# ak110/object_detector

Hardware: AMD Instinct MI355X
Metric: images_per_sec (higher is better)
Workload: dtype f16

## Files before the change

object_detector_amd/csrc/conv_8ph_kernel.h:

```cpp
#pragma once
#include "conv_8ph_tile.h"
#include "conv_common.h"

namespace {

constexpr int E_ALO = 0, E_AHI = E_REGION, E_BLO = 2 * E_REGION, E_BHI = 3 * E_REGION;

struct TapWalk {
  int c0, tap, tapoff, dx;
  int sel_tap;
};

constexpr unsigned E_OOB = 0x80000000u;

template <int MT, int NF = 4, bool KEEP = false>
static __device__ __forceinline__ void e8_epilogue_rt(const ConvKP& p, f32x4 (&acc)[MT][NF], int m0w, int n0w, int l15,
                                                          int lq, f16x8 (*keep)[NF / 2] = nullptr, int mrows = MT * 16,
                                                          const float* pre_sc = nullptr, const float* pre_bi = nullptr) {
  unsigned pb[MT], ppix[MT];
#pragma unroll
  for (int i = 0; i < MT; ++i) {
    const int m = m0w + i * 16 + l15;
    pb[i] = (unsigned)m / (unsigned)p.HoWo;
    ppix[i] = (unsigned)m - pb[i] * (unsigned)p.HoWo;
  }
#pragma unroll
  for (int pr = 0; pr < NF / 2; ++pr) {
    const int n = n0w + (2 * pr + (lq & 1)) * 16 + (lq >> 1) * 8;
    const bool nok = n < p.Cout;
    float sc[8], bi[8];
    if (pre_sc) {
#pragma unroll
      for (int e = 0; e < 8; ++e) {
        sc[e] = pre_sc[e];
        bi[e] = pre_bi[e];
      }
    } else {
      const f32x4 s0 = *(const f32x4*)(p.scale + n), s1 = *(const f32x4*)(p.scale + n + 4);
      const f32x4 b0 = *(const f32x4*)(p.bias + n), b1 = *(const f32x4*)(p.bias + n + 4);
#pragma unroll
      for (int e = 0; e < 4; ++e) {
        sc[e] = s0[e];
        sc[4 + e] = s1[e];
        bi[e] = b0[e];
        bi[4 + e] = b1[e];
      }
    }
    f16x8 rv[MT];
#pragma unroll
    for (int i = 0; i < MT; ++i) {
      const int m = m0w + i * 16 + l15;
      f16x8 r = {0, 0, 0, 0, 0, 0, 0, 0};
      if (nok && m < p.M && p.res_mode != OD_RES_NONE) {
        long long roff;
        if (p.res_mode == OD_RES_SAME) {
          roff = (long long)m * p.Cout + n;
        } else {
          const unsigned ho = ppix[i] / (unsigned)p.Wo, wo = ppix[i] - ho * (unsigned)p.Wo;
          roff = ((long long)(pb[i] * (unsigned)(p.Ho >> 1) + (ho >> 1)) * (p.Wo >> 1) + (wo >> 1)) * p.Cout + n;
        }
        r = *(const f16x8*)(p.res + roff);
      }
      rv[i] = r;
    }
#pragma unroll
    for (int i = 0; i < MT; ++i) {
      const int m = m0w + i * 16 + l15;
      const bool ok = nok && m < p.M && i * 16 + l15 < mrows;
      float v[8];
#pragma unroll
      for (int e = 0; e < 4; ++e) {
        float a = acc[i][2 * pr][e], bq = acc[i][2 * pr + 1][e];
        od_permlane16_swap(a, bq);
        v[e] = a;
        v[4 + e] = bq;
      }
#pragma unroll
      for (int e = 0; e < 8; ++e) v[e] = v[e] * sc[e] + bi[e];
      if (p.act == OD_ACT_LEAKY) {
#pragma unroll
        for (int e = 0; e < 8; ++e) v[e] = od_leaky(v[e], p.alpha);
      } else if (p.act == OD_ACT_ELU) {
#pragma unroll
        for (int e = 0; e < 8; ++e) v[e] = v[e] > 0.f ? v[e] : p.alpha * od_expm1_fast(v[e]);
      }
      if (p.res_mode != OD_RES_NONE) {
#pragma unroll
        for (int e = 0; e < 8; ++e) v[e] += (float)rv[i][e];
      }
      if (ok) {
        const long long ooff = (long long)pb[i] * p.obs + (long long)ppix[i] * p.ops + n;
        if (p.out_f32) {
          float* o = (float*)p.out + ooff;
          *(f32x4*)o = f32x4{v[0], v[1], v[2], v[3]};
          *(f32x4*)(o + 4) = f32x4{v[4], v[5], v[6], v[7]};
        } else {
          f16x8 h;
#pragma unroll
          for (int e = 0; e < 8; ++e) h[e] = (f16)v[e];
          *(f16x8*)((f16*)p.out + ooff) = h;
        }
      }
      if (KEEP) {
        f16x8 h;
#pragma unroll
        for (int e = 0; e < 8; ++e) h[e] = (f16)v[e];
        keep[i][pr] = h;
      }
    }
  }
}

template <int EPI, int MT, int NF, bool KEEP>
static __device__ __forceinline__ void e8_epilogue_fixed(const ConvKP& p, f32x4 (&acc)[MT][NF], int m0w, int n0w, int l15, int lq,
                                                         f16x8 (*keep)[NF / 2], int mrows, const float* pre_sc,
                                                         const float* pre_bi) {
  constexpr int ACT = od_epi_act(EPI), RES = od_epi_res(EPI);
  constexpr bool F32 = od_epi_f32(EPI);
  unsigned orow[MT], rrow[RES != OD_RES_NONE ? MT : 1];
#pragma unroll
  for (int i = 0; i < MT; ++i) {
    const unsigned m = (unsigned)min(m0w + i * 16 + l15, p.M - 1);
    const unsigned b = m / (unsigned)p.HoWo, pix = m - b * (unsigned)p.HoWo;
    orow[i] = b * (unsigned)p.obs + pix * (unsigned)p.ops;
    if (RES == OD_RES_SAME) rrow[i] = m * (unsigned)p.Cout;
    if (RES == OD_RES_UP2) {
      const unsigned ho = pix / (unsigned)p.Wo, wo = pix - ho * (unsigned)p.Wo;
      rrow[i] = ((b * (unsigned)(p.Ho >> 1) + (ho >> 1)) * (unsigned)(p.Wo >> 1) + (wo >> 1)) * (unsigned)p.Cout;
    }
  }
#pragma unroll
  for (int pr = 0; pr < NF / 2; ++pr) {
    const int n = n0w + (2 * pr + (lq & 1)) * 16 + (lq >> 1) * 8;
    const bool nok = n < p.Cout;
    float sc[8], bi[8];
    if (pre_sc) {
#pragma unroll
      for (int e = 0; e < 8; ++e) {
        sc[e] = pre_sc[e];
        bi[e] = pre_bi[e];
      }
    } else {
      const f32x4 s0 = *(const f32x4*)(p.scale + n), s1 = *(const f32x4*)(p.scale + n + 4);
      const f32x4 b0 = *(const f32x4*)(p.bias + n), b1 = *(const f32x4*)(p.bias + n + 4);
#pragma unroll
      for (int e = 0; e < 4; ++e) {
        sc[e] = s0[e];
        sc[4 + e] = s1[e];
        bi[e] = b0[e];
        bi[4 + e] = b1[e];
      }
    }
    f16x8 rv[RES != OD_RES_NONE ? MT : 1];
    if (RES != OD_RES_NONE) {
      const unsigned nr = nok ? (unsigned)n : 0u;
#pragma unroll
      for (int i = 0; i < MT; ++i) rv[i] = *(const f16x8*)(p.res + (rrow[i] + nr));
    }
#pragma unroll
    for (int i = 0; i < MT; ++i) {
      f32x4 a = acc[i][2 * pr], bq = acc[i][2 * pr + 1];
      od_permlane16_swap4(a, bq);
      float v[8] = {a[0], a[1], a[2], a[3], bq[0], bq[1], bq[2], bq[3]};
#pragma unroll
      for (int e = 0; e < 8; ++e) v[e] = v[e] * sc[e] + bi[e];
      if (ACT == OD_ACT_LEAKY) {
#pragma unroll
        for (int e = 0; e < 8; ++e) v[e] = od_leaky(v[e], p.alpha);
      } else if (ACT == OD_ACT_ELU) {
#pragma unroll
        for (int e = 0; e < 8; ++e) v[e] = od_elu_select(v[e], p.alpha);
      }
      if (RES != OD_RES_NONE) {
#pragma unroll
        for (int e = 0; e < 8; ++e) v[e] += (float)rv[i][e];
      }
      f16x8 h;
      if (!F32 || KEEP) {
#pragma unroll
        for (int e = 0; e < 8; ++e) h[e] = (f16)v[e];
      }
      if (nok && m0w + i * 16 + l15 < p.M && i * 16 + l15 < mrows) {
        const unsigned ooff = orow[i] + (unsigned)n;
        if (F32) {
          float* o = (float*)p.out + ooff;
          *(f32x4*)o = f32x4{v[0], v[1], v[2], v[3]};
          *(f32x4*)(o + 4) = f32x4{v[4], v[5], v[6], v[7]};
        } else {
          *(f16x8*)((f16*)p.out + ooff) = h;
        }
      }
      if (KEEP) keep[i][pr] = h;
    }
  }
}

template <int MT, int NF = 4, bool KEEP = false, int EPI = OD_EPI_RT>
static __device__ __forceinline__ void e8_epilogue_direct(const ConvKP& p, f32x4 (&acc)[MT][NF], int m0w, int n0w, int l15,
                                                          int lq, f16x8 (*keep)[NF / 2] = nullptr, int mrows = MT * 16,
                                                          const float* pre_sc = nullptr, const float* pre_bi = nullptr) {
  if constexpr (EPI == OD_EPI_RT)
    e8_epilogue_rt<MT, NF, KEEP>(p, acc, m0w, n0w, l15, lq, keep, mrows, pre_sc, pre_bi);
  else
    e8_epilogue_fixed<EPI, MT, NF, KEEP>(p, acc, m0w, n0w, l15, lq, keep, mrows, pre_sc, pre_bi);
}

template <int KS, int MF1, int EPI, int EPI2, bool PW, bool SEG>
__global__ __launch_bounds__(512, 2) void od_conv_8ph(ConvKP p_in) {
  constexpr int MF0 = 4, MT = MF0 + MF1, WROWS = MT * 16, BM = 2 * WROWS;
  extern __shared__ __attribute__((aligned(16))) char smem[];
  const int tid = threadIdx.x;
  const int lane = tid & 63;
  const int wave = __builtin_amdgcn_readfirstlane(tid >> 6);
  const int wr = wave >> 2, wc = wave & 3;
  const int l15 = lane & 15, lq = lane >> 4;

  int logical;
  {
    const int nt = p_in.mtiles * p_in.ntiles;
    const int pid = p_in.splitk > 1 ? (int)blockIdx.x / p_in.splitk : (int)blockIdx.x;
    const int q = nt >> 3, r = nt & 7, xcd = pid & 7, loc = pid >> 3;
    logical = (xcd < r ? xcd * (q + 1) : r * (q + 1) + (xcd - r) * q) + loc;
  }
  int tm = logical / p_in.ntiles;
  const int tn = logical - tm * p_in.ntiles;
  ConvKP p_seg;
  if (SEG) p_seg = p_in;
  if (SEG && p_in.nseg > 1) {
    int sg = 0;
    if (tm >= p_in.seg_tile0[1]) sg = 1;
    if (p_in.nseg > 2 && tm >= p_in.seg_tile0[2]) sg = 2;
    tm -= p_in.seg_tile0[sg];
    p_seg.x = p_in.seg_x[sg];
    p_seg.out = p_in.seg_out[sg];
    p_seg.H = p_seg.Ho = p_in.seg_H[sg];
    p_seg.W = p_seg.Wo = p_in.seg_W[sg];
    p_seg.HoWo = p_seg.H * p_seg.W;
    p_seg.M = p_in.seg_M[sg];
    p_seg.x_bytes = (unsigned)p_seg.M * (unsigned)p_in.Cin * 2u;
    if (p_in.obs == 0) p_seg.obs = (long long)p_seg.HoWo * p_in.Cout;
  }
  const ConvKP& p = SEG ? p_seg : p_in;
  const int m0 = tm * BM, n0 = tn * E_BN;
  const int nk_all = p.Ktot / E_BK;
  const int ks0 = p.splitk > 1 ? ((int)blockIdx.x % p.splitk) * p.steps_per_split : 0;
  const int nk = p.splitk > 1 ? min(p.steps_per_split, nk_all - ks0) : nk_all;
  if (nk <= 0) return;

  const int rr = tid >> 3;
  const int lc = (tid & 7) ^ (rr & 7);
  int a_base[2][2];
  unsigned a_vmask[2][2];
  unsigned a_sel[2][2];
#pragma unroll
  for (int s = 0; s < 2; ++s)
#pragma unroll
    for (int j = 0; j < 2; ++j) {
      const int m = m0 + j * WROWS + s * 64 + rr;
      a_vmask[s][j] = 0u;
      a_base[s][j] = 0;
      if (m < p.M && (s == 0 || rr < MF1 * 16)) {
        const unsigned b = (unsigned)m / (unsigned)p.HoWo;
        const unsigned pix = (unsigned)m - b * (unsigned)p.HoWo;
        const unsigned ho = pix / (unsigned)p.Wo;
        const unsigned wo = pix - ho * (unsigned)p.Wo;
        const int hi0 = (int)ho * p.stride - p.pad, wi0 = (int)wo * p.stride - p.pad;
        a_base[s][j] = ((((int)b * p.H + hi0 + p.pad) * p.W + wi0 + p.pad) * p.Cin + lc * 8) * 2;
#pragma unroll
        for (int t = 0; t < KS * KS; ++t) {
          const int hi = hi0 + t / KS, wi = wi0 + t % KS;
          if ((unsigned)hi < (unsigned)p.H && (unsigned)wi < (unsigned)p.W) a_vmask[s][j] |= 1u << t;
        }
      }
    }
  int w_off[2][2];
#pragma unroll
  for (int s = 0; s < 2; ++s)
#pragma unroll
    for (int j = 0; j < 2; ++j) {
      const int n = n0 + (2 * j + (rr >> 5)) * 64 + s * 32 + (rr & 31);
      w_off[s][j] = (n * p.Kstride + lc * 8 + ks0 * E_BK) * 2;
    }
  const __amdgpu_buffer_rsrc_t rs_x = __builtin_amdgcn_make_buffer_rsrc(
      (void*)(p.x - (long long)p.pad * (p.W + 1) * p.Cin), 0, (int)(p.x_bytes + (unsigned)(p.pad * (p.W + 1) * p.Cin * 2)),
      0x00020000);
  const __amdgpu_buffer_rsrc_t rs_w = __builtin_amdgcn_make_buffer_rsrc((void*)p.w, 0, (int)p.w_bytes, 0x00020000);
  auto blds16 = [&](const __amdgpu_buffer_rsrc_t& rs, unsigned voff, int soff, char* lptr) {
    __builtin_amdgcn_raw_ptr_buffer_load_lds(rs, (__attribute__((address_space(3))) void*)lptr, 16, (int)voff, soff, 0, 0);
  };

  auto walk_init = [&](TapWalk& w, int kt) {
    const int k0 = kt * E_BK;
    if (KS == 3) {
      w.sel_tap = -1;
      w.tap = k0 / p.Cin;
      w.c0 = k0 - w.tap * p.Cin;
      const int dy = w.tap / 3;
      w.dx = w.tap - dy * 3;
      w.tapoff = (dy * p.W + w.dx) * p.Cin;
    } else {
      w.sel_tap = -1;
      w.tap = 0;
      w.c0 = k0;
      w.dx = 0;
      w.tapoff = 0;
    }
  };
  auto walk_next = [&](TapWalk& w) {
    w.c0 += E_BK;
    if (KS == 3 && w.c0 >= p.Cin) {
      w.c0 = 0;
      ++w.tap;
      if (++w.dx == 3) {
        w.dx = 0;
        w.tapoff += (p.W - 2) * p.Cin;
      } else {
        w.tapoff += p.Cin;
      }
    }
  };
  TapWalk walk_lo, walk_hi;
  walk_init(walk_lo, ks0);
  walk_init(walk_hi, ks0);

  char* const piece = smem + wave * 1024;
  auto stage_a = [&](int s, TapWalk& w, int buf) {
    const int koff = w.tapoff + w.c0;
    char* dst = piece + buf * E_BUF + (s ? E_AHI : E_ALO);
    if (w.sel_tap != w.tap) {
      w.sel_tap = w.tap;
#pragma unroll
      for (int j = 0; j < 2; ++j) a_sel[s][j] = ((a_vmask[s][j] >> w.tap) & 1u) ? (unsigned)a_base[s][j] : E_OOB;
    }
#pragma unroll
    for (int j = 0; j < 2; ++j) blds16(rs_x, a_sel[s][j], koff * 2, dst + j * 8192);
    walk_next(w);
  };
  auto stage_b = [&](int s, int t, int buf) {
    char* dst = piece + buf * E_BUF + (s ? E_BHI : E_BLO);
#pragma unroll
    for (int j = 0; j < 2; ++j) blds16(rs_w, (unsigned)w_off[s][j], t * (E_BK * 2), dst + j * 8192);
  };

  const int w2buf = ((nk - 1) & 1) ^ 1;
  const __amdgpu_buffer_rsrc_t rs_w2 =
      __builtin_amdgcn_make_buffer_rsrc((void*)(PW ? p.w2 : p.w), 0, (int)(PW ? p.w2_bytes : p.w_bytes), 0x00020000);
  auto stage_w2 = [&](int ks) {
#pragma unroll
    for (int h = 0; h < 2; ++h)
      blds16(rs_w2, (unsigned)(((h * 64 + rr) * p.K2stride + lc * 8) * 2), ks * (E_BK * 2),
             piece + w2buf * E_BUF + ks * E_REGION + h * 8192);
  };

  f32x4 acc[MT][4];
#pragma unroll
  for (int i = 0; i < MT; ++i)
#pragma unroll
    for (int j = 0; j < 4; ++j) acc[i][j] = f32x4{0.f, 0.f, 0.f, 0.f};

  stage_a(0, walk_lo, 0);
  stage_b(0, 0, 0);
  stage_b(1, 0, 0);
  stage_a(1, walk_hi, 0);
  if (nk > 1) {
    stage_a(0, walk_lo, 1);
    stage_b(0, 1, 1);
    wait_vmcnt<8>();
  } else {
    wait_vmcnt<0>();
  }
  __builtin_amdgcn_s_barrier();

  const int fa = (wr * 64 + l15) * 128 + ((lq ^ (l15 & 7)) * 16);
  const int fb = (wc * 32 + l15) * 128 + ((lq ^ (l15 & 7)) * 16);

  f16x8 xa[MF0][2], wlo[2][2], whi[2][2];
  auto ldf = [&](f16x8& dst, const char* src) { dst = *(const f16x8*)src; };
  auto mma = [&](f32x4& c, const f16x8& a, const f16x8& b) {
    c = __builtin_amdgcn_mfma_f32_16x16x32_f16(a, b, c, 0, 0, 0);
  };

  auto L0 = [&](int t) {
    const char* cur = smem + (t & 1) * E_BUF;
#pragma unroll
    for (int f = 0; f < 2; ++f)
#pragma unroll
      for (int kh = 0; kh < 2; ++kh) ldf(wlo[f][kh], cur + E_BLO + ((fb + f * 2048) ^ (kh * 64)));
#pragma unroll
    for (int f = 0; f < MF0; ++f)
#pragma unroll
      for (int kh = 0; kh < 2; ++kh) ldf(xa[f][kh], cur + E_ALO + ((fa + f * 2048) ^ (kh * 64)));
    if (t + 1 < nk) {
      stage_b(1, t + 1, (t & 1) ^ 1);
      wait_vmcnt<8>();
    } else if (PW) {
      stage_w2(0);
      wait_vmcnt<2>();
    } else {
      wait_vmcnt<0>();
    }
  };
  auto L1 = [&](int t) {
    const char* cur = smem + (t & 1) * E_BUF;
#pragma unroll
    for (int f = 0; f < 2; ++f)
#pragma unroll
      for (int kh = 0; kh < 2; ++kh) ldf(whi[f][kh], cur + E_BHI + ((fb + f * 2048) ^ (kh * 64)));
    if (t + 1 < nk) {
      stage_a(1, walk_hi, (t & 1) ^ 1);
      wait_vmcnt<8>();
    } else if (PW) {
      stage_w2(1);
    } else {
      wait_vmcnt<0>();
    }
  };
  auto L2 = [&](int t) {
    const char* cur = smem + (t & 1) * E_BUF;
#pragma unroll
    for (int f = 0; f < MF1; ++f)
#pragma unroll
      for (int kh = 0; kh < 2; ++kh) ldf(xa[f][kh], cur + E_AHI + ((fa + f * 2048) ^ (kh * 64)));
    if (t + 2 < nk) stage_a(0, walk_lo, t & 1);
    if (PW && t + 1 == nk) stage_w2(2);
  };
  auto L3 = [&](int t) {
    if (t + 2 < nk) {
      stage_b(0, t + 2, t & 1);
      wait_vmcnt<8>();
    } else if (PW && t + 1 == nk) {
      stage_w2(3);
    } else {
      wait_vmcnt<0>();
    }
  };
  auto M = [&](int ph) {
    __builtin_amdgcn_s_setprio(1);
#pragma unroll
    for (int kh = 0; kh < 2; ++kh)
#pragma unroll
      for (int i = 0; i < ((ph < 2) ? MF0 : MF1); ++i)
#pragma unroll
        for (int j = 0; j < 2; ++j) {
          if (ph == 0) mma(acc[i][j], wlo[j][kh], xa[i][kh]);
          if (ph == 1) mma(acc[i][2 + j], whi[j][kh], xa[i][kh]);
          if (ph == 2) mma(acc[MF0 + i][2 + j], whi[j][kh], xa[i][kh]);
          if (ph == 3) mma(acc[MF0 + i][j], wlo[j][kh], xa[i][kh]);
        }
    __builtin_amdgcn_s_setprio(0);
  };

  if (wr == 0) {
    for (int t = 0; t < nk; ++t) {
      L0(t);
      M(0);
      __builtin_amdgcn_s_barrier();
      L1(t);
      M(1);
      __builtin_amdgcn_s_barrier();
      L2(t);
      M(2);
      __builtin_amdgcn_s_barrier();
      L3(t);
      M(3);
      __builtin_amdgcn_s_barrier();
    }
  } else {
    L0(0);
    __builtin_amdgcn_s_barrier();
    for (int t = 0; t < nk; ++t) {
      M(0);
      L1(t);
      __builtin_amdgcn_s_barrier();
      M(1);
      L2(t);
      __builtin_amdgcn_s_barrier();
      M(2);
      L3(t);
      __builtin_amdgcn_s_barrier();
      M(3);
      if (t + 1 < nk) {
        L0(t + 1);
        __builtin_amdgcn_s_barrier();
      }
    }
  }
  __syncthreads();

  if constexpr (PW) {
    const int rg = wave >> 2, cg = wave & 3;
    float sc2[8], bi2[8];
    {
      const int n2 = cg * 32 + (lq & 1) * 16 + (lq >> 1) * 8;
      const f32x4 s0 = *(const f32x4*)(p.scale2 + n2), s1 = *(const f32x4*)(p.scale2 + n2 + 4);
      const f32x4 b0 = *(const f32x4*)(p.bias2 + n2), b1 = *(const f32x4*)(p.bias2 + n2 + 4);
#pragma unroll
      for (int e = 0; e < 4; ++e) {
        sc2[e] = s0[e];
        sc2[4 + e] = s1[e];
        bi2[e] = b0[e];
        bi2[4 + e] = b1[e];
      }
    }
    f16x8 ykeep[MT][2];
    od_mfma_results_ready();
    e8_epilogue_direct<MT, 4, true, EPI>(p, acc, m0 + wr * WROWS, n0 + wc * 64, l15, lq, ykeep);
    ConvKP p2 = p;
    p2.scale = p.scale2;
    p2.bias = p.bias2;
    p2.act = p.act2;
    p2.alpha = p.alpha2;
    p2.res_mode = OD_RES_NONE;
    p2.out = (void*)p.out2;
    p2.out_f32 = 0;
    p2.Cout = p.Cout2;
    p2.obs = (long long)p.HoWo * p.Cout2;
    p2.ops = p.Cout2;
    char* const ybuf = smem + (w2buf ^ 1) * E_BUF;
    const char* const wbuf = smem + w2buf * E_BUF;
    const int fy = (rg * 64 + l15) * 128 + ((lq ^ (l15 & 7)) * 16);
    const int fw = (cg * 32 + l15) * 128 + ((lq ^ (l15 & 7)) * 16);
#pragma unroll
    for (int half = 0; half < 2; ++half) {
      if (wr == half) {
#pragma unroll
        for (int i = 0; i < MT; ++i)
#pragma unroll
          for (int pr = 0; pr < 2; ++pr) {
            const int row = i * 16 + l15;
            const int chunk = (2 * pr + (lq & 1)) * 2 + (lq >> 1);
            *(f16x8*)(ybuf + wc * E_REGION + row * 128 + ((chunk ^ (row & 7)) * 16)) = ykeep[i][pr];
          }
      }
      asm volatile("s_waitcnt lgkmcnt(0)" ::: "memory");
      __builtin_amdgcn_s_barrier();
      f32x4 acc2[4][2];
#pragma unroll
      for (int i = 0; i < 4; ++i)
#pragma unroll
        for (int f = 0; f < 2; ++f) acc2[i][f] = f32x4{0.f, 0.f, 0.f, 0.f};
#pragma unroll
      for (int ks = 0; ks < 4; ++ks)
#pragma unroll
        for (int kh = 0; kh < 2; ++kh) {
          f16x8 wf[2], yf[4];
#pragma unroll
          for (int f = 0; f < 2; ++f) wf[f] = *(const f16x8*)(wbuf + ks * E_REGION + ((fw + f * 2048) ^ (kh * 64)));
#pragma unroll
          for (int i = 0; i < 4; ++i) yf[i] = *(const f16x8*)(ybuf + ks * E_REGION + ((fy + i * 2048) ^ (kh * 64)));
#pragma unroll
          for (int i = 0; i < 4; ++i)
#pragma unroll
            for (int f = 0; f < 2; ++f) acc2[i][f] = __builtin_amdgcn_mfma_f32_16x16x32_f16(wf[f], yf[i], acc2[i][f], 0, 0, 0);
        }
      od_mfma_results_ready();
      e8_epilogue_direct<4, 2, false, EPI2>(p2, acc2, m0 + half * WROWS + rg * 64, cg * 32, l15, lq, nullptr, WROWS - rg * 64, sc2, bi2);
      if (half == 0) {
        asm volatile("s_waitcnt lgkmcnt(0)" ::: "memory");
        __builtin_amdgcn_s_barrier();
      }
    }
  } else if (EPI == OD_EPI_RT && p.splitk > 1) {
    conv_epilogue<E_BN, 2, 4, MT, 4, 512>(p, smem, acc, m0, n0, tid, wr, wc, l15, lq);
  } else {
    od_mfma_results_ready();
    e8_epilogue_direct<MT, 4, false, EPI>(p, acc, m0 + wr * WROWS, n0 + wc * 64, l15, lq);
  }
}

}
```

object_detector_amd/csrc/conv_common.h:

```cpp
#pragma once
#include "common.h"

struct ConvKP {
  const f16* x;
  const f16* w;
  const float* scale;
  const float* bias;
  const f16* res;
  void* out;
  const f16* zero;
  int H, W, Cin, Ho, Wo, Cout;
  int stride, pad;
  int Kstride, Ktot, M, HoWo;
  int act;
  float alpha;
  int res_mode, out_f32;
  long long obs, ops;
  int mtiles, ntiles;
  int splitk, steps_per_split;
  float* ws;
  int Mq;
  int tconv, Hs, Ws;
  unsigned x_bytes, w_bytes;
  float* stats;
  const f16* w2;
  const float* scale2;
  const float* bias2;
  f16* out2;
  int Cout2, act2;
  float alpha2;
  unsigned w2_bytes;
  int K2stride;
  int nseg;
  int seg_tile0[4];
  const f16* seg_x[3];
  void* seg_out[3];
  int seg_H[3], seg_W[3], seg_M[3];
  int off32;
};

static __device__ __forceinline__ void glds16(const void* gptr, void* lptr) {
  __builtin_amdgcn_global_load_lds((const __attribute__((address_space(1))) void*)gptr,
                                   (__attribute__((address_space(3))) void*)lptr, 16, 0, 0);
}

static __device__ __forceinline__ float od_expm1_fast(float v) {
  const float poly = v * (1.f + v * (0.5f + v * (1.f / 6 + v * (1.f / 24 + v * (1.f / 120 + v * (1.f / 720))))));
  return v > -0.25f ? poly : __expf(v) - 1.f;
}

static __device__ __forceinline__ float od_elu_select(float v, float alpha) {
  const float poly = v * (1.f + v * (0.5f + v * (1.f / 6 + v * (1.f / 24 + v * (1.f / 120 + v * (1.f / 720))))));
  const float ex = __expf(v) - 1.f;
  const float em = v > -0.25f ? poly : ex;
  const float neg = alpha * em;
  return v > 0.f ? v : neg;
}

#define OD_EPI_RT -1
#define OD_EPI_LEAKY_NONE_F16 1
#define OD_EPI_LEAKY_SAME_F16 5
#define OD_EPI_ELU_NONE_F16 2
#define OD_EPI_ELU_UP2_F16 10
#define OD_EPI_LINEAR_NONE_F32 16
#define OD_EPI_LEAKY_NONE_F32 17
#define OD_EPI_ELU_NONE_F32 18
constexpr int od_epi(int act, int res_mode, bool out_f32) { return act | (res_mode << 2) | ((int)out_f32 << 4); }
static_assert(od_epi(OD_ACT_LEAKY, OD_RES_NONE, false) == OD_EPI_LEAKY_NONE_F16 &&
                  od_epi(OD_ACT_LEAKY, OD_RES_SAME, false) == OD_EPI_LEAKY_SAME_F16 &&
                  od_epi(OD_ACT_ELU, OD_RES_NONE, false) == OD_EPI_ELU_NONE_F16 &&
                  od_epi(OD_ACT_ELU, OD_RES_UP2, false) == OD_EPI_ELU_UP2_F16 &&
                  od_epi(OD_ACT_LINEAR, OD_RES_NONE, true) == OD_EPI_LINEAR_NONE_F32 &&
                  od_epi(OD_ACT_LEAKY, OD_RES_NONE, true) == OD_EPI_LEAKY_NONE_F32 &&
                  od_epi(OD_ACT_ELU, OD_RES_NONE, true) == OD_EPI_ELU_NONE_F32,
              "OD_EPI_* literals");
constexpr int od_epi_act(int epi) { return epi & 3; }
constexpr int od_epi_res(int epi) { return (epi >> 2) & 3; }
constexpr bool od_epi_f32(int epi) { return ((epi >> 4) & 1) != 0; }
static inline int od_epi_of(const ConvKP& p) {
  return (p.off32 && p.splitk <= 1 && !p.tconv && !p.stats) ? od_epi(p.act, p.res_mode, p.out_f32 != 0) : OD_EPI_RT;
}
#define OD_STR_(x) #x
#define OD_STR(x) OD_STR_(x)

static __device__ __forceinline__ void od_permlane16_swap(float& a, float& b) {
  asm volatile("s_nop 1\n\tv_permlane16_swap_b32 %0, %1\n\ts_nop 1" : "+v"(a), "+v"(b));
}
static __device__ __forceinline__ void od_permlane16_swap4(f32x4& a, f32x4& b) {
  float a0 = a[0], a1 = a[1], a2 = a[2], a3 = a[3], b0 = b[0], b1 = b[1], b2 = b[2], b3 = b[3];
  asm volatile(
      "s_nop 1\n\tv_permlane16_swap_b32 %0, %4\n\tv_permlane16_swap_b32 %1, %5\n\tv_permlane16_swap_b32 %2, %6\n\t"
      "v_permlane16_swap_b32 %3, %7\n\ts_nop 1"
      : "+v"(a0), "+v"(a1), "+v"(a2), "+v"(a3), "+v"(b0), "+v"(b1), "+v"(b2), "+v"(b3));
  a = f32x4{a0, a1, a2, a3};
  b = f32x4{b0, b1, b2, b3};
}
static __device__ __forceinline__ void od_mfma_results_ready() {
  __builtin_amdgcn_sched_barrier(0);
  asm volatile("s_nop 15\n\ts_nop 15" ::: "memory");
  __builtin_amdgcn_sched_barrier(0);
}

static __device__ __forceinline__ float od_leaky(float v, float alpha) { return fmaxf(v, v * alpha); }

template <int N>
static __device__ __forceinline__ void wait_vmcnt() {
  asm volatile("s_waitcnt vmcnt(%0)" ::"n"(N) : "memory");
}


static __device__ __forceinline__ int od_tconv_pixel(const ConvKP& p, unsigned m, unsigned BM) {
  const unsigned t = m / BM, r = m - t * BM;
  const unsigned cls = t & 3u, idx = (t >> 2) * BM + r;
  if (idx >= (unsigned)p.Mq) return -1;
  const unsigned HsWs = (unsigned)(p.Hs * p.Ws);
  const unsigned b = idx / HsWs, q = idx - b * HsWs;
  const unsigned i = q / (unsigned)p.Ws, j = q - i * (unsigned)p.Ws;
  return (int)(b * (unsigned)p.HoWo + (2u * i + (cls >> 1)) * (unsigned)p.Wo + 2u * j + (cls & 1u));
}

template <int BN, int WM, int WN, int MT, int NTL, int NT = WM * WN * 64, bool STATS = false, int EPI = OD_EPI_RT>
static __device__ __forceinline__ void conv_epilogue(const ConvKP& p, char* smem, f32x4 (&acc)[MT][NTL], int m0, int n0,
                                                     int tid, int wm, int wn, int l15, int lq) {
  constexpr int WTM = MT * 16, WTN = NTL * 16, SLD = BN + 4;
  constexpr bool FX = EPI != OD_EPI_RT;
  static_assert(!(FX && STATS), "the statistics epilogue has no policy");
  const int act = FX ? od_epi_act(EPI) : p.act, res_mode = FX ? od_epi_res(EPI) : p.res_mode;
  const bool out_f32 = FX ? od_epi_f32(EPI) : p.out_f32 != 0;
  const bool splitk = !FX && p.splitk > 1, tconv = !FX && p.tconv;
  float* stg = (float*)smem;
  constexpr int CH = BN / 8;
  constexpr int RPP = NT / CH;
  const int c8 = (tid % CH) * 8;
  const int n = n0 + c8;
  float sc[8], bi[8];
  if (!STATS) {
    const f32x4 s0 = *(const f32x4*)(p.scale + n), s1 = *(const f32x4*)(p.scale + n + 4);
    const f32x4 b0 = *(const f32x4*)(p.bias + n), b1 = *(const f32x4*)(p.bias + n + 4);
#pragma unroll
    for (int e = 0; e < 4; ++e) {
      sc[e] = s0[e];
      sc[4 + e] = s1[e];
      bi[e] = b0[e];
      bi[4 + e] = b1[e];
    }
  }
  float st0[STATS ? 8 : 1], st1[STATS ? 8 : 1];
  if (STATS) {
#pragma unroll
    for (int e = 0; e < 8; ++e) st0[e] = st1[e] = 0.f;
  }
  constexpr int NPASS = (WTM + RPP - 1) / RPP;
  constexpr bool RAGGED = (WTM % RPP) != 0;
  f16x8 resv[WM][NPASS];
  if (res_mode != OD_RES_NONE && !splitk) {
#pragma unroll
    for (int wr = 0; wr < WM; ++wr)
#pragma unroll
      for (int ps = 0; ps < NPASS; ++ps) {
        int m = m0 + wr * WTM + ps * RPP + tid / CH;
        f16x8 r = {0, 0, 0, 0, 0, 0, 0, 0};
        if (RAGGED && ps * RPP + tid / CH >= WTM) m = p.M;
        if (tconv && m < p.M) m = od_tconv_pixel(p, (unsigned)m, WM * MT * 16);
        if (m >= 0 && m < p.M && n < p.Cout) {
          long long roff;
          if (res_mode == OD_RES_SAME) {
            roff = (long long)m * p.Cout + n;
          } else {
            const unsigned b = (unsigned)m / (unsigned)p.HoWo;
            const unsigned pix = (unsigned)m - b * (unsigned)p.HoWo;
            const unsigned ho = pix / (unsigned)p.Wo, wo = pix - ho * (unsigned)p.Wo;
            roff = ((long long)(b * (unsigned)(p.Ho >> 1) + (ho >> 1)) * (p.Wo >> 1) + (wo >> 1)) * p.Cout + n;
          }
          r = *(const f16x8*)(p.res + roff);
        }
        resv[wr][ps] = r;
      }
  }
#pragma unroll
  for (int wr = 0; wr < WM; ++wr) {
    if (wm == wr) {
#pragma unroll
      for (int j = 0; j < NTL; ++j) {
        const int nl = wn * WTN + j * 16 + lq * 4;
#pragma unroll
        for (int i = 0; i < MT; ++i) *(f32x4*)(stg + (i * 16 + l15) * SLD + nl) = acc[i][j];
      }
    }
    __syncthreads();
    if (splitk) {
      float* slab = p.ws + (long long)((int)blockIdx.x % p.splitk) * p.M * p.Cout;
#pragma unroll
      for (int ps = 0; ps < NPASS; ++ps) {
        const int row = ps * RPP + tid / CH;
        const int m = (RAGGED && row >= WTM) ? p.M : m0 + wr * WTM + row;
        if (m < p.M && n < p.Cout) {
          float* o = slab + (long long)m * p.Cout + n;
          *(f32x4*)o = *(const f32x4*)(stg + row * SLD + c8);
          *(f32x4*)(o + 4) = *(const f32x4*)(stg + row * SLD + c8 + 4);
        }
      }
      if (wr + 1 < WM) __syncthreads();
      continue;
    }
#pragma unroll
    for (int ps = 0; ps < NPASS; ++ps) {
      const int row = ps * RPP + tid / CH;
      int m = (RAGGED && row >= WTM) ? p.M : m0 + wr * WTM + row;
      if (tconv && m < p.M) m = od_tconv_pixel(p, (unsigned)m, WM * MT * 16);
      if (m >= 0 && m < p.M && n < p.Cout) {
        const f32x4 v0 = *(const f32x4*)(stg + row * SLD + c8);
        const f32x4 v1 = *(const f32x4*)(stg + row * SLD + c8 + 4);
        float v[8] = {v0[0], v0[1], v0[2], v0[3], v1[0], v1[1], v1[2], v1[3]};
        if (!STATS) {
#pragma unroll
          for (int e = 0; e < 8; ++e) v[e] = v[e] * sc[e] + bi[e];
        }
        if (STATS) {
        } else if (act == OD_ACT_LEAKY) {
#pragma unroll
          for (int e = 0; e < 8; ++e) v[e] = od_leaky(v[e], p.alpha);
        } else if (act == OD_ACT_ELU) {
#pragma unroll
          for (int e = 0; e < 8; ++e) v[e] = FX ? od_elu_select(v[e], p.alpha) : (v[e] > 0.f ? v[e] : p.alpha * od_expm1_fast(v[e]));
        }
        if (!STATS && res_mode != OD_RES_NONE) {
#pragma unroll
          for (int e = 0; e < 8; ++e) v[e] += (float)resv[wr][ps][e];
        }
        const unsigned b = (unsigned)m / (unsigned)p.HoWo;
        const unsigned pix = (unsigned)m - b * (unsigned)p.HoWo;
        const long long ooff = FX ? (long long)(b * (unsigned)p.obs + pix * (unsigned)p.ops + (unsigned)n)
                                  : (long long)b * p.obs + (long long)pix * p.ops + n;
        if (out_f32) {
          float* o = (float*)p.out + ooff;
          *(f32x4*)o = f32x4{v[0], v[1], v[2], v[3]};
          *(f32x4*)(o + 4) = f32x4{v[4], v[5], v[6], v[7]};
        } else {
          f16x8 h;
#pragma unroll
          for (int e = 0; e < 8; ++e) h[e] = (f16)v[e];
          *(f16x8*)((f16*)p.out + ooff) = h;
          if (STATS) {
#pragma unroll
            for (int e = 0; e < 8; ++e) {
              const float q = (float)h[e];
              st0[e] += q;
              st1[e] += q * q;
            }
          }
        }
      }
    }
    if (wr + 1 < WM) __syncthreads();
  }
  if (STATS) {
    static_assert(CH == 8 || CH == 16 || CH == 32, "BN must be 64, 128 or 256");
#pragma unroll
    for (int off = CH; off < 64; off <<= 1) {
#pragma unroll
      for (int e = 0; e < 8; ++e) {
        st0[e] += __shfl_xor(st0[e], off, 64);
        st1[e] += __shfl_xor(st1[e], off, 64);
      }
    }
    __syncthreads();
    float* red = (float*)smem;
    const int wv = tid >> 6, ln = tid & 63;
    if (ln < CH) {
#pragma unroll
      for (int e = 0; e < 8; ++e) {
        red[(wv * CH + ln) * 16 + e] = st0[e];
        red[(wv * CH + ln) * 16 + 8 + e] = st1[e];
      }
    }
    __syncthreads();
    if (tid < CH && n < p.Cout) {
      float a[8], b[8];
#pragma unroll
      for (int e = 0; e < 8; ++e) a[e] = b[e] = 0.f;
      for (int w2 = 0; w2 < NT / 64; ++w2) {
#pragma unroll
        for (int e = 0; e < 8; ++e) {
          a[e] += red[(w2 * CH + tid) * 16 + e];
          b[e] += red[(w2 * CH + tid) * 16 + 8 + e];
        }
      }
      float* row = p.stats + (long long)(m0 / (WM * WTM)) * 2 * p.Cout;
#pragma unroll
      for (int e = 0; e < 8; ++e) {
        row[n + e] = a[e];
        row[p.Cout + n + e] = b[e];
      }
    }
  }
}

struct ConvKernelInfo {
  const void* fn;
  const char* name;
  int BM, BN, BK, threads;
  size_t lds;
};

int od_conv_igemm_num_cfgs();
bool od_conv_igemm_select(int cfg, int ksize, int Cin, bool want_stats, int epi, ConvKernelInfo* info);
int od_conv_finish_prepare(const ConvKP& p, od_launches* L);
int od_conv_8ph_num_cfgs();
long od_conv_8ph_tiles(int idx, int M, int Cout);
double od_conv_8ph_tile_cost(int idx, int nk);
bool od_conv_8ph_can_fuse_pointwise(const ConvKP& p);
bool od_conv_8ph_select(int idx, const ConvKP& p, int ksize, ConvKernelInfo* info);
bool od_conv_8ph_variant_mf4(int ksize, bool pw, int epi, int epi2, const void** fn, const char** name);
bool od_conv_8ph_variant_mf3(int ksize, bool pw, int epi, int epi2, const void** fn, const char** name);
bool od_conv_8ph_variant_mf2(int ksize, bool pw, int epi, int epi2, const void** fn, const char** name);
bool od_conv_8ph_variant_mf1(int ksize, bool pw, int epi, int epi2, const void** fn, const char** name);
bool od_tconv_small_supported(const od_conv_desc* d);
int od_tconv_small_prepare(od_ctx* ctx, const od_conv_desc* d, od_launches* L);
bool od_conv_rdirect_supported(const od_conv_desc* d);
int od_conv_rdirect_prepare(od_ctx* ctx, const od_conv_desc* d, od_launches* L);
bool od_conv_stream3_supported(const od_conv_desc* d);
int od_conv_stream3_prepare(od_ctx* ctx, const od_conv_desc* d, od_launches* L);
```

Baseline: 22600.

## Restructure fixed epilogue to hoist scale/bias/residual loads ahead of compute

New measurement: 22790 (median of 6 runs). About the same (+0.9%).

```diff
diff --git a/object_detector_amd/csrc/conv_8ph_kernel.h b/object_detector_amd/csrc/conv_8ph_kernel.h
--- a/object_detector_amd/csrc/conv_8ph_kernel.h
+++ b/object_detector_amd/csrc/conv_8ph_kernel.h
@@ -115,84 +115,140 @@
 static __device__ __forceinline__ void e8_epilogue_fixed(const ConvKP& p, f32x4 (&acc)[MT][NF], int m0w, int n0w, int l15, int lq,
                                                          f16x8 (*keep)[NF / 2], int mrows, const float* pre_sc,
                                                          const float* pre_bi) {
-  constexpr int ACT = od_epi_act(EPI), RES = od_epi_res(EPI);
-  constexpr bool F32 = od_epi_f32(EPI);
-  unsigned orow[MT], rrow[RES != OD_RES_NONE ? MT : 1];
+  constexpr int ACT = od_epi_act(EPI), RES = od_epi_res(EPI), NP = NF / 2;
+  constexpr bool F32 = od_epi_f32(EPI), HASRES = RES != OD_RES_NONE;
+  constexpr int NP0 = (HASRES && KEEP) ? 1 : NP;
+  static_assert(!(F32 && (HASRES || KEEP)), "f32 outputs have no residual and no fused consumer");
+  unsigned rrow[HASRES ? MT : 1];
+  if (HASRES) {
+#pragma unroll
+    for (int i = 0; i < MT; ++i) {
+      const unsigned m = (unsigned)min(m0w + i * 16 + l15, p.M - 1);
+      if (RES == OD_RES_SAME) rrow[i] = m * (unsigned)p.Cout;
+      if (RES == OD_RES_UP2) {
+        const unsigned b = m / (unsigned)p.HoWo, pix = m - b * (unsigned)p.HoWo;
+        const unsigned ho = pix / (unsigned)p.Wo, wo = pix - ho * (unsigned)p.Wo;
+        rrow[i] = ((b * (unsigned)(p.Ho >> 1) + (ho >> 1)) * (unsigned)(p.Wo >> 1) + (wo >> 1)) * (unsigned)p.Cout;
+      }
+    }
+  }
+  int n[NP];
+  float sc[NP][8], bi[NP][8];
+  f16x8 rv[HASRES ? NP : 1][HASRES ? MT : 1];
+#pragma unroll
+  for (int pr = 0; pr < NP; ++pr) n[pr] = n0w + (2 * pr + (lq & 1)) * 16 + (lq >> 1) * 8;
+  auto load_scale_bias = [&](int pr) {
+    if (pre_sc) {
+#pragma unroll
+      for (int e = 0; e < 8; ++e) {
+        sc[pr][e] = pre_sc[e];
+        bi[pr][e] = pre_bi[e];
+      }
+    } else {
+      const f32x4 s0 = *(const f32x4*)(p.scale + n[pr]), s1 = *(const f32x4*)(p.scale + n[pr] + 4);
+      const f32x4 b0 = *(const f32x4*)(p.bias + n[pr]), b1 = *(const f32x4*)(p.bias + n[pr] + 4);
+#pragma unroll
+      for (int e = 0; e < 4; ++e) {
+        sc[pr][e] = s0[e];
+        sc[pr][4 + e] = s1[e];
+        bi[pr][e] = b0[e];
+        bi[pr][4 + e] = b1[e];
+      }
+    }
+  };
+#pragma unroll
+  for (int pr = 0; pr < NP0; ++pr) load_scale_bias(pr);
+  auto load_res = [&](int pr, int i) {
+    const unsigned nr = n[pr] < p.Cout ? (unsigned)n[pr] : 0u;
+    rv[pr][i] = *(const f16x8*)(p.res + (rrow[i] + nr));
+  };
+  if (HASRES) {
+#pragma unroll
+    for (int pr = 0; pr < NP0; ++pr)
+#pragma unroll
+      for (int i = 0; i < MT; ++i) load_res(pr, i);
+  }
+  const bool loads = !pre_sc || HASRES;
+  float v[NP][MT][8];
+  if (loads) __builtin_amdgcn_sched_barrier(0);
+  auto swap_row = [&](int pr, int i) {
+    f32x4 a = acc[i][2 * pr], bq = acc[i][2 * pr + 1];
+    od_permlane16_swap4(a, bq);
+#pragma unroll
+    for (int e = 0; e < 4; ++e) {
+      v[pr][i][e] = a[e];
+      v[pr][i][4 + e] = bq[e];
+    }
+  };
+  constexpr bool SWAP_EARLY = NP0 == NP;
+  if (SWAP_EARLY) {
+#pragma unroll
+    for (int pr = 0; pr < NP; ++pr)
+#pragma unroll
+      for (int i = 0; i < MT; ++i) swap_row(pr, i);
+  }
+  if (loads) od_loads_retired();
+  f16x8 h[F32 ? 1 : NP][F32 ? 1 : MT];
+#pragma unroll
+  for (int pr = 0; pr < NP; ++pr) {
+    if (pr >= NP0) od_loads_retired();
+#pragma unroll
+    for (int i = 0; i < MT; ++i) {
+      if (!SWAP_EARLY) swap_row(pr, i);
+      float(&w)[8] = v[pr][i];
+#pragma unroll
+      for (int e = 0; e < 8; ++e) w[e] = w[e] * sc[pr][e] + bi[pr][e];
+      if (ACT == OD_ACT_LEAKY) {
+#pragma unroll
+        for (int e = 0; e < 8; ++e) w[e] = od_leaky(w[e], p.alpha);
+      } else if (ACT == OD_ACT_ELU) {
+#pragma unroll
+        for (int e = 0; e < 8; ++e) w[e] = od_elu_select(w[e], p.alpha);
+      }
+      if (HASRES) {
+#pragma unroll
+        for (int e = 0; e < 8; ++e) w[e] += (float)rv[pr][i][e];
+      }
+      if (!F32) {
+#pragma unroll
+        for (int e = 0; e < 8; ++e) h[pr][i][e] = (f16)w[e];
+        if (KEEP) {
+          asm volatile("" : "+v"(h[pr][i]));
+          keep[i][pr] = h[pr][i];
+        }
+      }
+      if (pr + 1 >= NP0 && pr + 1 < NP) {
+        if (i == 1) load_scale_bias(pr + 1);
+        load_res(pr + 1, i);
+      }
+    }
+  }
+  __builtin_amdgcn_sched_barrier(0);
+  int l15s = l15;
+  asm volatile("" : "+v"(l15s));
+  const int rows = min(p.M - m0w, mrows) - l15s;
+  unsigned orow[MT];
 #pragma unroll
   for (int i = 0; i < MT; ++i) {
-    const unsigned m = (unsigned)min(m0w + i * 16 + l15, p.M - 1);
+    const unsigned m = (unsigned)min(m0w + i * 16 + l15s, p.M - 1);
     const unsigned b = m / (unsigned)p.HoWo, pix = m - b * (unsigned)p.HoWo;
     orow[i] = b * (unsigned)p.obs + pix * (unsigned)p.ops;
-    if (RES == OD_RES_SAME) rrow[i] = m * (unsigned)p.Cout;
-    if (RES == OD_RES_UP2) {
-      const unsigned ho = pix / (unsigned)p.Wo, wo = pix - ho * (unsigned)p.Wo;
-      rrow[i] = ((b * (unsigned)(p.Ho >> 1) + (ho >> 1)) * (unsigned)(p.Wo >> 1) + (wo >> 1)) * (unsigned)p.Cout;
-    }
-  }
-#pragma unroll
-  for (int pr = 0; pr < NF / 2; ++pr) {
-    const int n = n0w + (2 * pr + (lq & 1)) * 16 + (lq >> 1) * 8;
-    const bool nok = n < p.Cout;
-    float sc[8], bi[8];
-    if (pre_sc) {
-#pragma unroll
-      for (int e = 0; e < 8; ++e) {
-        sc[e] = pre_sc[e];
-        bi[e] = pre_bi[e];
-      }
-    } else {
-      const f32x4 s0 = *(const f32x4*)(p.scale + n), s1 = *(const f32x4*)(p.scale + n + 4);
-      const f32x4 b0 = *(const f32x4*)(p.bias + n), b1 = *(const f32x4*)(p.bias + n + 4);
-#pragma unroll
-      for (int e = 0; e < 4; ++e) {
-        sc[e] = s0[e];
-        sc[4 + e] = s1[e];
-        bi[e] = b0[e];
-        bi[4 + e] = b1[e];
-      }
-    }
-    f16x8 rv[RES != OD_RES_NONE ? MT : 1];
-    if (RES != OD_RES_NONE) {
-      const unsigned nr = nok ? (unsigned)n : 0u;
-#pragma unroll
-      for (int i = 0; i < MT; ++i) rv[i] = *(const f16x8*)(p.res + (rrow[i] + nr));
-    }
+  }
+#pragma unroll
+  for (int pr = 0; pr < NP; ++pr)
 #pragma unroll
     for (int i = 0; i < MT; ++i) {
-      f32x4 a = acc[i][2 * pr], bq = acc[i][2 * pr + 1];
-      od_permlane16_swap4(a, bq);
-      float v[8] = {a[0], a[1], a[2], a[3], bq[0], bq[1], bq[2], bq[3]};
-#pragma unroll
-      for (int e = 0; e < 8; ++e) v[e] = v[e] * sc[e] + bi[e];
-      if (ACT == OD_ACT_LEAKY) {
-#pragma unroll
-        for (int e = 0; e < 8; ++e) v[e] = od_leaky(v[e], p.alpha);
-      } else if (ACT == OD_ACT_ELU) {
-#pragma unroll
-        for (int e = 0; e < 8; ++e) v[e] = od_elu_select(v[e], p.alpha);
-      }
-      if (RES != OD_RES_NONE) {
-#pragma unroll
-        for (int e = 0; e < 8; ++e) v[e] += (float)rv[i][e];
-      }
-      f16x8 h;
-      if (!F32 || KEEP) {
-#pragma unroll
-        for (int e = 0; e < 8; ++e) h[e] = (f16)v[e];
-      }
-      if (nok && m0w + i * 16 + l15 < p.M && i * 16 + l15 < mrows) {
-        const unsigned ooff = orow[i] + (unsigned)n;
+      if (n[pr] < p.Cout && i * 16 < rows) {
+        const unsigned ooff = orow[i] + (unsigned)n[pr];
         if (F32) {
           float* o = (float*)p.out + ooff;
-          *(f32x4*)o = f32x4{v[0], v[1], v[2], v[3]};
-          *(f32x4*)(o + 4) = f32x4{v[4], v[5], v[6], v[7]};
+          *(f32x4*)o = f32x4{v[pr][i][0], v[pr][i][1], v[pr][i][2], v[pr][i][3]};
+          *(f32x4*)(o + 4) = f32x4{v[pr][i][4], v[pr][i][5], v[pr][i][6], v[pr][i][7]};
         } else {
-          *(f16x8*)((f16*)p.out + ooff) = h;
+          *(f16x8*)((f16*)p.out + ooff) = h[pr][i];
         }
       }
-      if (KEEP) keep[i][pr] = h;
-    }
-  }
+    }
 }
 
 template <int MT, int NF = 4, bool KEEP = false, int EPI = OD_EPI_RT>
diff --git a/object_detector_amd/csrc/conv_common.h b/object_detector_amd/csrc/conv_common.h
--- a/object_detector_amd/csrc/conv_common.h
+++ b/object_detector_amd/csrc/conv_common.h
@@ -107,6 +107,11 @@
 static __device__ __forceinline__ void wait_vmcnt() {
   asm volatile("s_waitcnt vmcnt(%0)" ::"n"(N) : "memory");
 }
+static __device__ __forceinline__ void od_loads_retired() {
+  __builtin_amdgcn_sched_barrier(0);
+  __builtin_amdgcn_s_waitcnt(0x0F70);
+  __builtin_amdgcn_sched_barrier(0);
+}
 
 
 static __device__ __forceinline__ int od_tconv_pixel(const ConvKP& p, unsigned m, unsigned BM) {
@@ -188,6 +193,7 @@
       }
     }
     __syncthreads();
+    if (FX && wr == 0) od_loads_retired();
     if (splitk) {
       float* slab = p.ws + (long long)((int)blockIdx.x % p.splitk) * p.M * p.Cout;
 #pragma unroll
```
